# HKU-BAL/MegaPath-Nano

Measured on AMD Instinct MI355X. Metric: Gbp/min ONT reads aligned+species-assigned vs RefSeq, 1/2/4/8 MI355X, higher is better.
Workload: dtype int32

## Files before the change

### megapath_nano_amd/csrc/align.hip

```cpp
#include "map_types.h"
#include "ext_kernels.h"
#include "fin_kernels.h"
#include "stitch_kernels.h"
#include "plan_kernels.h"
#include "hit_kernels.h"
#include "mapper_internal.h"
#include "../../include/mpn_map.h"
#include "../../include/mpn_ssw.h"

#include <algorithm>
#include <condition_variable>
#include <deque>
#include <math.h>
#include <stdio.h>
#include <string.h>
#include <thread>
#include <pthread.h>
#include <time.h>
#include <atomic>
#include <functional>
#include <mutex>
#include <stdlib.h>
#include <string>
#include <vector>
// ... 762 lines not shown
    int nj = nj_cap;
    WallTimer wt;
    Slot &SL = *tl_slot;
    const int strip_scores = ext_strip_scores_ok(opt->a, -opt->b, -opt->sc_ambi, opt->q + opt->e, opt->q2 + opt->e2) ? 1 : 0;
    ExtParams prm;
    prm.sc_mch = (int8_t)opt->a; prm.sc_mis = (int8_t)-opt->b; prm.sc_n = (int8_t)-opt->sc_ambi;
    prm.q = (int8_t)opt->q; prm.e = (int8_t)opt->e; prm.q2 = (int8_t)opt->q2; prm.e2 = (int8_t)opt->e2; prm.zdrop_thres = opt->zdrop;
    prm.zdrop_inv = opt->zdrop_inv; prm.max_gap = opt->max_gap;
    const size_t order_cap = (size_t)nj + (size_t)N_STRIP * 8 + 16;
    if (SL.pool_sizes.ensure((size_t)nj * sizeof(JobSizes) + 16) || SL.pool_buckets.ensure((size_t)2 * N_BUCKETS * 4 + sizeof(LayoutTotals) + 16) ||
        SL.pool_order.ensure(order_cap * 4) || SL.pin_res.ensure(sizeof(LayoutTotals) + 96) ||
        SL.pool_redo_ids.ensure((size_t)nj * 4 + 16) || SL.pool_probes.ensure((size_t)nj * sizeof(InvProbe) + 16))
        return -1;
    struct { ExtJob *p; } d_jobs{dv.jobs};
    JobSizes *d_sizes = SL.pool_sizes.as<JobSizes>();
    int32_t *d_bcnt = SL.pool_buckets.as<int32_t>(), *d_bcur = d_bcnt + N_BUCKETS;
    LayoutTotals *d_tot = reinterpret_cast<LayoutTotals *>(d_bcnt + 2 * N_BUCKETS);
    struct { int32_t *p; } d_order{SL.pool_order.as<int32_t>()};
    {
        ZeroList z{};
        zero_list_push(z, d_bcnt, (size_t)2 * N_BUCKETS * 4 + sizeof(LayoutTotals));
        zero_list_push(z, dv.used + 1, 8);
        zero_list_push(z, dv.used + 5, 8);
        zero_list_push(z, dv.used + 7, 8);
        MPN_HIP_CHECK(zero_regions(z, st));
    }
    const int lay_grid = std::max(1, std::min((nj + 255) / 256, 256));
    EvTimer evl(st);
    static const bool tiled_on = []() { const char *e = getenv("MPN_TILED"); return !e || atoi(e) != 0; }();
    static const int tile_pick = []() { const char *e = getenv("MPN_TILE_CLASS"); return e ? std::min(std::max(atoi(e), 0), N_TILE_CLASS - 1) : -1; }();
    hipLaunchKernelGGL(job_classify_kernel, dim3(lay_grid), dim3(256), 0, st, d_jobs.p, d_nj, strip_scores, prm, g_force_kernel ? g_force_kernel : (tiled_on ? 0 : 7),
                       tile_pick, d_sizes, d_bcnt, d_tot);
    hipLaunchKernelGGL(job_scan_kernel, dim3(1), dim3(1024), 0, st, d_sizes, d_nj, (const int32_t *)d_bcnt, d_bcur, d_tot, d_order.p);
    hipLaunchKernelGGL(job_layout_kernel, dim3(lay_grid), dim3(256), 0, st, d_jobs.p, d_nj, (const JobSizes *)d_sizes, d_bcur, d_order.p);
    MPN_HIP_CHECK(hipGetLastError());
    LayoutTotals *h_tot = SL.pin_res.as<LayoutTotals>();
    evl.mark(56);
    MPN_HIP_CHECK(hipMemcpyAsync(h_tot, d_tot, sizeof(LayoutTotals), hipMemcpyDeviceToHost, st));
    MPN_HIP_CHECK(stream_sync(st));
    evl.resolve();
    const LayoutTotals T = *h_tot;
    nj = T.n_jobs;
    dv.n_jobs = nj;
    if (nj == 0) return 0;
    if (T.too_large) { set_error("DP window too large for LDS staging (%d x %d)", T.tl_q, T.tl_t); return -4; }
    if (!dv.compact) {
// ... 123 lines not shown
    EvTimer ev(st);
    if (!SL.ev_b) {
        MPN_HIP_CHECK(hipEventCreateWithFlags(&SL.ev_b, hipEventDisableTiming));
        MPN_HIP_CHECK(hipEventCreateWithFlags(&SL.ev_c, hipEventDisableTiming));
    }
    auto on_side = [](int l) { return (l >= L_WG && l < L_STRIP) || l >= L_BAND + 8; };
    bool have_tiles = false;
    for (int l = L_TILE; l < N_LISTS; ++l) have_tiles = have_tiles || cnt[l] > 0;
    bool have_side = false;
    for (int l = 0; l < L_TILE; ++l) have_side = have_side || (on_side(l) && cnt[l] > 0);
    hipStream_t extra[2] = {nullptr, nullptr};
    const int n_extra = st.try_extra((int)have_side + (int)have_tiles, extra);
    if (have_side || have_tiles) ++g_stats[n_extra ? STAT_SIDE_LEASED : STAT_SIDE_OWN];
    const hipStream_t main_st = st;
    const hipStream_t side_st = have_side && n_extra > 0 ? extra[0] : main_st;
    const hipStream_t tile_st = have_tiles && n_extra > (int)have_side ? extra[(int)have_side] : main_st;
    for (int l = L_TILE; l < N_LISTS && have_tiles; ++l)
        if (launch_list(l, d_order.p + base[l], cnt[l], tile_st)) return -1;
    for (int l = L_TILE - 1; l >= 0; --l)
        if (on_side(l) && launch_list(l, d_order.p + base[l], cnt[l], side_st)) return -1;
    const int side_lo[2] = {base[L_WG], base[L_BAND + 8]}, side_hi[2] = {base[L_STRIP], base[L_TILE]};
    const int tile_lo[2] = {base[L_TILE], 0}, tile_hi[2] = {base[N_LISTS], 0};
    const int main_lo[2] = {0, base[L_STRIP]}, main_hi[2] = {base[L_WG], base[L_BAND + 8]};
    auto bt_ztest = [&](const int *lo, const int *hi, hipStream_t s, bool timed) -> int {
        for (int k = 0; k < 2; ++k) {
            const int n = hi[k] - lo[k];
            if (n > 0) hipLaunchKernelGGL(ext_bt_kernel, dim3((n + 63) / 64), dim3(64), 0, s, d_jobs.p, d_order.p + lo[k], n, P.p, OFF.p, CIG.p, d_compact, d_used, d_res.p);
        }
        MPN_HIP_CHECK(hipGetLastError());
        if (timed) ev.mark(25);
        for (int k = 0; k < 2; ++k) {
            const int n = hi[k] - lo[k];
            if (n > 0) hipLaunchKernelGGL(ext_ztest_kernel, dim3((n + 63) / 64), dim3(64), 0, s, d_jobs.p, d_order.p + lo[k], n, prm, d_reads, d_read_off, d_read_len, rv, CIG.p, d_res.p,
                                          d_redo_ids, d_used + 1, d_probes, d_used + 5);
        }
        MPN_HIP_CHECK(hipGetLastError());
        if (timed) ev.mark(26);
        return 0;
    };
    if (have_tiles) {
        if (bt_ztest(tile_lo, tile_hi, tile_st, false)) return -1;
        if (tile_st != main_st) MPN_HIP_CHECK(hipEventRecord(SL.ev_c, tile_st));
    }
    if (bt_ztest(side_lo, side_hi, side_st, false)) return -1;
    if (side_st != main_st) MPN_HIP_CHECK(hipEventRecord(SL.ev_b, side_st));
    for (int l = N_LISTS - 1; l >= 0; --l) {
        if (on_side(l)) continue;
        if (l == L_BAND - 1) ev.mark(15);
        if (l >= L_STRIP && l < L_BAND) {
            if (l == L_STRIP + 48) { if (launch_list(l, nullptr, 1, main_st)) return -1; ev.mark(57); }
            else if (l == L_STRIP) { if (launch_list(l, nullptr, 1, main_st)) return -1; ev.mark(9, 38); }
        } else if (launch_list(l, d_order.p + base[l], cnt[l], main_st)) return -1;
    }
    ev.mark(15);
    if (bt_ztest(main_lo, main_hi, main_st, true)) return -1;
    if (side_st != main_st) MPN_HIP_CHECK(hipStreamWaitEvent(main_st, SL.ev_b, 0));
    if (tile_st != main_st) MPN_HIP_CHECK(hipStreamWaitEvent(main_st, SL.ev_c, 0));
    unsigned long long *h_used = reinterpret_cast<unsigned long long *>(reinterpret_cast<char *>(SL.pin_res.p) + ((sizeof(LayoutTotals) + 15) & ~(size_t)15));
    MPN_HIP_CHECK(hipMemcpyAsync(h_used, d_used, 64, hipMemcpyDeviceToHost, st));
    wt.stop_into(g_stats[28]);
    MPN_HIP_CHECK(stream_sync(st));
    wt.stop_into(g_stats[29]);
    if (h_used[7]) {
        g_stats[STAT_TILE_GIVEUPS] += (int64_t)h_used[7];
        set_error("%llu tiled DP windows gave up waiting for their hand-off", (unsigned long long)h_used[7]);
        return -1;
    }
    std::vector<int32_t> redo((size_t)h_used[1]);
    const int n_probe = (int)h_used[5];
    if (!redo.empty() || n_probe) {
        std::vector<ExtJob> jobs((size_t)nj);
        std::vector<InvProbe> probes((size_t)n_probe);
        if (SL.pin_order.ensure(redo.size() * 4 + 16)) return -1;
        if (!redo.empty()) MPN_HIP_CHECK(hipMemcpyAsync(SL.pin_order.p, d_redo_ids, redo.size() * 4, hipMemcpyDeviceToHost, st));
        MPN_HIP_CHECK(hipMemcpyAsync(jobs.data(), d_jobs.p, (size_t)nj * sizeof(ExtJob), hipMemcpyDeviceToHost, st));
        if (n_probe) MPN_HIP_CHECK(hipMemcpyAsync(probes.data(), d_probes, (size_t)n_probe * sizeof(InvProbe), hipMemcpyDeviceToHost, st));
        MPN_HIP_CHECK(stream_sync(st));
        if (!redo.empty()) memcpy(redo.data(), SL.pin_order.p, redo.size() * 4);
        std::vector<uint8_t> is_inv((size_t)nj, 0);
        if (n_probe) {
            std::sort(probes.begin(), probes.end(), [](const InvProbe &x, const InvProbe &y) { return x.jid < y.jid; });
            std::vector<LocalHit> hits((size_t)n_probe, LocalHit{0, -1, -1});
            if (hs) {
                std::vector<std::vector<int8_t>> qv((size_t)n_probe), tv;
                std::vector<RefIv> iv((size_t)n_probe);
// ... 35 lines not shown
                const int64_t n_r = (int64_t)jb.qlen + jb.tlen - 1;
                pack_off[k] = -1 - p2_tot;
                p2_tot += ((bv >= 0 ? n_r * (128 << bv) : n_r * jb.n_col) + 15) & ~(int64_t)15;
            } else pack_off[k] = jb.p_off;
        }
        if (nr > 0) {
            if (SL.pool_P2.ensure((size_t)p2_tot + 16)) return -1;
            const int64_t p2_base = (int64_t)(SL.pool_P2.as<uint8_t>() - P.p);
            for (int k = 0; k < nr; ++k) if (pack_off[k] < 0) pack_off[k] = p2_base + (-1 - pack_off[k]);
            if (SL.pool_redo.ensure(pack.size() * 4)) return -1;
            struct { int32_t *p; } d_redo{SL.pool_redo.as<int32_t>()};
            MPN_HIP_CHECK(hipMemcpyAsync(d_redo.p, pack.data(), pack.size() * 4, hipMemcpyHostToDevice, st));
            hipLaunchKernelGGL(ext_redo_patch_kernel, dim3((nr + 255) / 256), dim3(256), 0, st, d_jobs.p, d_redo.p, d_redo.p + nr, d_redo.p + 2 * nr,
                               reinterpret_cast<const int64_t *>(d_redo.p + off_p), d_redo.p + 3 * nr, opt->zdrop_inv, nr);
            MPN_HIP_CHECK(hipGetLastError());
            ev.skip();
            for (int lo = 0; lo < nr;) {
                int hi = lo;
                while (hi < nr && redo_list_of(redo[hi]) == redo_list_of(redo[lo])) ++hi;
                if (launch_list(redo_list_of(redo[lo]), d_redo.p + lo, hi - lo, st)) return -1;
                lo = hi;
            }
            ev.mark(15);
            hipLaunchKernelGGL(ext_bt_kernel, dim3((nr + 63) / 64), dim3(64), 0, st, d_jobs.p, d_redo.p, nr, P.p, OFF.p, CIG.p, d_compact, d_used, d_res.p);
            MPN_HIP_CHECK(hipGetLastError());
            ev.mark(25);
            MPN_HIP_CHECK(stream_sync(st));
        }
    }
    ev.resolve();
    wt.stop_into(g_stats[30]);
    return 0;
}

static int run_jobs(const RefView &rv, const mpn_map_opt *opt, int nj_cap, const uint8_t *d_reads, const int64_t *d_read_off,
                    const int32_t *d_read_len, DevRound &out, const HostSeqs *hs, StreamLease &st, bool block_zeroed = false) {
    static const int64_t budget = []() { const char *e = getenv("MPN_DP_BUDGET"); return e ? std::max<int64_t>(1 << 20, atoll(e)) : (int64_t)40 << 30; }();
    Slot &SL = *tl_slot;
    if (SL.pool_res.ensure((size_t)nj_cap * sizeof(ExtRes) + 16) || SL.pool_used.ensure(128)) return -1;
    out.jobs = SL.pool_jobs.as<ExtJob>(); out.res = SL.pool_res.as<ExtRes>(); out.compact = nullptr;
    out.used = SL.pool_used.as<unsigned long long>();
    if (!block_zeroed) {
        MPN_HIP_CHECK(hipMemsetAsync(out.used, 0, 24, st));
        MPN_HIP_CHECK(hipMemsetAsync(out.used + 5, 0, 24, st));
    }
    const int rc = run_job_group(rv, opt, nj_cap, out.used + 3, out, d_reads, d_read_off, d_read_len, budget, hs, st);
    if (rc != 1) return rc;
// ... 1133 lines not shown
    std::vector<int64_t> ns, ne;
    pack_2bit(tcodes, ttot, words, ns, ne);
    DevBuf<int32_t> d_qlen;
    if (d_reads.upload(ascii.data(), ascii.size(), st) || d_ref.upload(words.data(), words.size(), st) || d_ns.upload(ns.data(), ns.size(), st) ||
        d_ne.upload(ne.data(), ne.size(), st) || d_qoff.upload(q_off, n, st) ||
        d_qlen.upload(q_len, n, st) || d_toff.upload(t_off, n, st))
        return -1;
    std::vector<ExtJob> jobs(n);
    for (int i = 0; i < n; ++i) {
        ExtJob &j = jobs[i];
        memset(&j, 0, sizeof(j));
        j.read = i; j.rid = i; j.rev = 0; j.qs = 0; j.qlen = q_len[i]; j.ts = 0; j.tlen = t_len[i]; j.reversed = 0;
        j.w = w[i]; j.zdrop = zdrop[i]; j.end_bonus = end_bonus[i]; j.flag = flag[i];
    }
    g_force_kernel = force_kernel;
    mpn_map_opt o2 = *opt;
    o2.zdrop = 0x3fffffff;
    DevRound dv;
    for (ExtJob &j : jobs) { j.strip_s = 1; j.cls = -1; }
    if (tl_slot->pool_jobs.ensure((size_t)n * sizeof(ExtJob) + 16)) return -1;
    MPN_HIP_CHECK(hipMemcpy(tl_slot->pool_jobs.p, jobs.data(), (size_t)n * sizeof(ExtJob), hipMemcpyHostToDevice));
    {
        const unsigned long long cnt = (unsigned long long)n;
        if (tl_slot->pool_used.ensure(64)) return -1;
        MPN_HIP_CHECK(hipMemcpy(tl_slot->pool_used.as<unsigned long long>() + 3, &cnt, 8, hipMemcpyHostToDevice));
    }
    StreamLease sl(st);
    const int rc = run_jobs(RefView{d_ref.p, d_toff.p, d_ns.p, d_ne.p, (int32_t)ns.size()}, &o2, n, d_reads.p, d_qoff.p, d_qlen.p, dv, nullptr, sl);
    g_force_kernel = 0;
    if (rc) return rc;
    std::vector<ExtRes> res((size_t)n);
    unsigned long long h_used = 0;
    MPN_HIP_CHECK(hipMemcpy(res.data(), dv.res, (size_t)n * sizeof(ExtRes), hipMemcpyDeviceToHost));
    MPN_HIP_CHECK(hipMemcpy(&h_used, dv.used, 8, hipMemcpyDeviceToHost));
    std::vector<uint32_t> cig((size_t)h_used + 1);
    if (h_used) MPN_HIP_CHECK(hipMemcpy(cig.data(), dv.compact, (size_t)h_used * 4, hipMemcpyDeviceToHost));
    int64_t used = 0;
    for (int i = 0; i < n; ++i) {
        const ExtRes &e = res[i];
        int32_t *o = out9 + (size_t)i * 9;
        o[0] = e.max; o[1] = e.zdropped; o[2] = e.max_q; o[3] = e.max_t; o[4] = e.mqe; o[5] = e.mqe_t; o[6] = e.score; o[7] = e.reach_end;
        o[8] = e.n_cigar;
        cig_off[i] = used;
        if (used + e.n_cigar > cigar_cap) return -3;
        if (e.n_cigar) memcpy(cigar_pool + used, cig.data() + e.cig_pos, (size_t)e.n_cigar * 4);
        used += e.n_cigar;
    }
// ... 3 lines not shown
```

### megapath_nano_amd/csrc/ext_kernels.h

```cpp
#pragma once
#include "mpn_common.h"
#include "map_types.h"

namespace mpn {

enum { EZ_APPROX_MAX = 0x02, EZ_RIGHT = 0x08, EZ_EXTZ_ONLY = 0x40, EZ_REV_CIGAR = 0x80 };

struct ExtJob {
    int32_t read;
    int32_t rid;
    int32_t rev;
    int32_t qs, qlen;
    int32_t ts, tlen;
    int32_t reversed;
    int32_t w, zdrop, end_bonus, flag;
    int64_t p_off;
    int64_t row_off;
    int64_t cig_off;
    int32_t n_col;
    int32_t state_mode;
    int64_t state_off;
    int32_t layout;
    int32_t qstride;
    int32_t strip_s;
// ... 1265 lines not shown
            res[jid] = out;
        }
    }
}

template <int S, int NW>
__global__ __launch_bounds__(64 * NW) void ext_dp_tile_kernel(const ExtJob *__restrict__ jobs, const int32_t *__restrict__ order, int n_jobs,
                                                              ExtParams prm, const uint8_t *__restrict__ reads,
                                                              const int64_t *__restrict__ read_off, const int32_t *__restrict__ read_len,
                                                              RefView rv, uint8_t *__restrict__ P, int8_t *__restrict__ gstate, ExtRes *__restrict__ res,
                                                              unsigned long long *__restrict__ n_failed) {
    extern __shared__ __attribute__((aligned(16))) uint8_t smem[];
    const int jid = order[blockIdx.x];
    const ExtJob jb = jobs[jid];
#define MPN_TB(EX, RT) ext_tile_body<S, NW, EX, RT>(jb, jid, prm, reads, read_off, read_len, rv, P, gstate, res, smem, n_failed)
    if (jb.flag & EZ_APPROX_MAX) MPN_TB(false, false);
    else if (jb.flag & EZ_RIGHT) MPN_TB(true, true);
    else MPN_TB(true, false);
#undef MPN_TB
}



__global__ __launch_bounds__(64) void ext_bt_kernel(const ExtJob *__restrict__ jobs, const int32_t *__restrict__ order, int n_jobs,
                                                    const uint8_t *__restrict__ P, const int32_t *__restrict__ OFF,
                                                    uint32_t *__restrict__ CIG, uint32_t *__restrict__ COMPACT,
                                                    unsigned long long *__restrict__ compact_used, ExtRes *__restrict__ res) {
    const int k = blockIdx.x * blockDim.x + threadIdx.x;
    const int jid = k < n_jobs ? order[k] : -1;
    const bool live = jid >= 0;
    ExtJob jb = jobs[live ? jid : 0];
    ExtRes r = res[live ? jid : 0];
    const bool walk = live && r.do_bt;
    if (live && !r.do_bt) res[jid].cig_pos = 0;
    if (!walk) { jb.qlen = jb.tlen = 1; r.bt_i = r.bt_j = -1; }
    const int n_col = jb.n_col, n_r = jb.qlen + jb.tlen - 1;
    const uint8_t *p = P + jb.p_off;
    const int32_t *off = OFF + 2 * jb.row_off, *off_end = off + n_r;
    const bool rowmajor = jb.layout == 1;
    const bool rank_is_op = (jb.flag & EZ_RIGHT) != 0;
    const bool byslot = jb.layout == 2;
    const bool tiled = jb.layout == 3;
    TileGeom tg{};
    int tg_tile = -1;
    const int bw = jb.w < 0 ? (jb.tlen > jb.qlen ? jb.tlen : jb.qlen) : jb.w;
    const bool rev_cigar = (jb.flag & EZ_REV_CIGAR) != 0;
// ... 2 lines not shown
    uint32_t *cbeg = cend - cap;
    int n = 0, i = r.bt_i, j = r.bt_j, state = 0;
    uint32_t cur_op = 0xf, cur_len = 0;
#define MPN_FLUSH() do { if (cur_len) { if (rev_cigar) cbeg[n] = cur_len << 4 | cur_op; else cend[-1 - n] = cur_len << 4 | cur_op; ++n; } } while (0)
#define MPN_PUSHOP(OP, LEN) do { if ((uint32_t)(OP) == cur_op) cur_len += (LEN); else { MPN_FLUSH(); cur_op = (OP); cur_len = (LEN); } } while (0)
    constexpr int BT_AHEAD = 8;
    while (i >= 0 && j >= 0) {
        const int rr = i + j;
        int force_state = -1, tmp;
        if (rowmajor) {
            if (state == 0) {
                uint8_t ahead[BT_AHEAD];
#pragma unroll
                for (int k = 0; k < BT_AHEAD; ++k) {
                    const int ii = i - k, jj = j - k;
                    ahead[k] = (ii >= 0 && jj >= 0) ? p[(int64_t)(jj + ii / jb.strip_s) * jb.qstride + ii] : (uint8_t)0xff;
                }
                int k = 0;
                tmp = 0;
#pragma unroll
                for (int q = 0; q < BT_AHEAD; ++q) {
                    if (k != q) continue;
                    if (i - q < 0 || j - q < 0) continue;
                    int b = ahead[q];
                    if (!rank_is_op) b = (b & ~7) | (4 - (b & 7));
                    if ((b & 7) == 0) ++k; else tmp = b;
                }
                if (k > 0) { MPN_PUSHOP(0, (uint32_t)k); i -= k; j -= k; }
                if (k == BT_AHEAD || i < 0 || j < 0) continue;
            } else {
                tmp = p[(int64_t)(j + i / jb.strip_s) * jb.qstride + i];
                if (!rank_is_op) tmp = (tmp & ~7) | (4 - (tmp & 7));
            }
        }
        else if (tiled) {
            int st = 0, en = jb.tlen - 1;
            if (st < rr - jb.qlen + 1) st = rr - jb.qlen + 1;
            if (en > rr) en = rr;
            if (st < (rr - bw + 1) >> 1) st = (rr - bw + 1) >> 1;
            if (en > (rr + bw) >> 1) en = (rr + bw) >> 1;
            if (i < st) force_state = 2;
            if (i > en) force_state = 1;
            tmp = 0;
            if (force_state < 0) {
                const int tile = i / (64 * jb.strip_s);
                if (tile != tg_tile) { tg = tile_geom(tile, jb.qlen, jb.tlen, bw, jb.strip_s); tg_tile = tile; }
                const int lt = i - tg.T0;
                tmp = p[tg.base + (int64_t)((j - tg.jlo) + lt / jb.strip_s) * tg.W + lt];
                if (!rank_is_op) tmp = (tmp & ~7) | (4 - (tmp & 7));
            }
        }
        else if (byslot) {
            int st = 0, en = jb.tlen - 1;
            if (st < rr - jb.qlen + 1) st = rr - jb.qlen + 1;
            if (en > rr) en = rr;
            if (st < (rr - bw + 1) >> 1) st = (rr - bw + 1) >> 1;
            if (en > (rr + bw) >> 1) en = (rr + bw) >> 1;
            if (i < st) force_state = 2;
            if (i > en) force_state = 1;
            tmp = force_state < 0 ? p[(int64_t)rr * jb.qstride + (i & (jb.qstride - 1))] : 0;
        } else {
            if (i < off[rr]) force_state = 2;
            if (i > off_end[rr]) force_state = 1;
            tmp = force_state < 0 ? p[(int64_t)rr * n_col + i - off[rr]] : 0;
        }
        if (state == 0) state = tmp & 7;
        else if (!(tmp >> (state + 2) & 1)) state = 0;
        if (state == 0) state = tmp & 7;
        if (force_state >= 0) state = force_state;
        if (state == 0) { MPN_PUSHOP(0, 1); --i; --j; }
        else if (state == 1 || state == 3) { MPN_PUSHOP(2, 1); --i; }
        else { MPN_PUSHOP(1, 1); --j; }
    }
    if (walk) {
        if (i >= 0) MPN_PUSHOP(2, (uint32_t)(i + 1));
        if (j >= 0) MPN_PUSHOP(1, (uint32_t)(j + 1));
        MPN_FLUSH();
    }
#undef MPN_PUSHOP
#undef MPN_FLUSH
    const int lane = threadIdx.x & 63;
    int incl = n;
#pragma unroll
    for (int d = 1; d < 64; d <<= 1) { const int o = __shfl_up(incl, d); if (lane >= d) incl += o; }
    const int total = __shfl(incl, 63);
    unsigned long long base = 0;
    if (lane == 0 && total) base = atomicAdd(compact_used, (unsigned long long)total);
    base = (unsigned long long)__shfl((long long)base, 0);
    if (walk) {
        const unsigned long long pos = base + (unsigned long long)(incl - n);
        const uint32_t *src = rev_cigar ? cbeg : cend - n;
        for (int q = 0; q < n; ++q) COMPACT[pos + q] = src[q];
        res[jid].n_cigar = n;
        res[jid].cig_pos = (int64_t)pos;
    }
}

__global__ __launch_bounds__(64) void ext_ztest_kernel(const ExtJob *__restrict__ jobs, const int32_t *__restrict__ order, int n_jobs,
                                                       ExtParams prm, const uint8_t *__restrict__ reads,
                                                       const int64_t *__restrict__ read_off, const int32_t *__restrict__ read_len,
                                                       RefView rv,
                                                       const uint32_t *__restrict__ CIG, ExtRes *__restrict__ res,
                                                       int32_t *__restrict__ redo_ids, unsigned long long *__restrict__ n_redo,
                                                       InvProbe *__restrict__ probes, unsigned long long *__restrict__ n_probe) {
    const int k = blockIdx.x * blockDim.x + threadIdx.x;
    if (k >= n_jobs) return;
    const int jid = order[k];
    if (jid < 0) return;
    const ExtJob jb = jobs[jid];
    if (!(jb.flag & EZ_APPROX_MAX)) return;
    auto report = [&](int z) {
        res[jid].zcode = z;
        if (z) redo_ids[atomicAdd(n_redo, 1ULL)] = jid;
    };
    const ExtRes r = res[jid];
    const int zmin = prm.zdrop_thres < prm.zdrop_inv ? prm.zdrop_thres : prm.zdrop_inv;
    const uint32_t *cig = CIG + jb.cig_off - r.n_cigar;
    if ((jb.layout == 1 || jb.layout == 3) && r.do_bt && !r.zdropped) {
// ... 29 lines not shown
                } else { mx = score; max_i = i + l; max_j = j + l; }
            }
            i += len; j += len;
        } else if (op == 1 || op == 2) {
            score -= prm.q + prm.e * (int)len;
            if (op == 1) j += len; else i += len;
            if (score < mx) {
                const int li = i - max_i, lj = j - max_j, diff = li > lj ? li - lj : lj - li;
                const int z = mx - score - diff * prm.e;
                if (z > max_zdrop) { max_zdrop = z; p00 = max_i; p01 = max_j; p10 = i; p11 = j; }
            } else { mx = score; max_i = i; max_j = j; }
        }
    }
    const int over = max_zdrop > prm.zdrop_thres ? 1 : 0;
    const int q_len = p11 - p01, t_len = p10 - p00;
    if (max_zdrop > prm.zdrop_inv && q_len < prm.max_gap && t_len < prm.max_gap && q_len > 0 && t_len > 0) {
        res[jid].zcode = over;
        probes[atomicAdd(n_probe, 1ULL)] = InvProbe{jid, p00, p01, p10, p11, over};
        return;
    }
    report(over);
}

}
```

### megapath_nano_amd/csrc/mapper_internal.h

```cpp
#pragma once
#include "mpn_common.h"
#include "map_types.h"
#include "queue_lease.h"

#include <atomic>
#include <chrono>
#include <time.h>
#include <mutex>
#include <stdint.h>
#include <stdlib.h>
#include <string.h>
#include <string>
#include <vector>

struct mpn_map_opt_s;


struct mpn_index {
    int k = 15, w = 10;
    int32_t n_seq = 0;
    std::vector<std::string> names;
    std::vector<int32_t> lens;
    std::vector<int64_t> seq_off;
    std::vector<uint32_t> h_seq2;
// ... 28 lines not shown
    DevBuf<unsigned long long> used;
};

struct ReadSketch {
    DevBuf<int64_t> mz_off;
    DevBuf<u128> mz;
    int64_t n_mz = 0;
    int k = 0, w = 0;
    bool valid = false;
};

struct HostChains {
    std::vector<int64_t> n_anchor, chain_off, b_off;
    std::vector<int64_t> n_chained, u_pos, b_pos;
    std::vector<int32_t> n_chain, rep_len;
    const uint64_t *u_all = nullptr;
    const u128 *b_all = nullptr;
    const ChainRec *rec_all = nullptr;
    int64_t n_pool_chains = 0;
    void read_chains(int i, uint64_t *u_out, u128 *b_out) const;
    void chain_order(int i, int32_t *order, int64_t *src) const;
};

constexpr int MPN_NSTATS = 73;
constexpr int STAT_LEASE_WAIT = 65;
constexpr int STAT_SIDE_LEASED = 66, STAT_SIDE_OWN = 67;
constexpr int STAT_TILE_CLASS = 68, STAT_TILE_GIVEUPS = 72;
extern thread_local int64_t g_stats[MPN_NSTATS];

void pack_2bit(const uint8_t *codes, int64_t n, std::vector<uint32_t> &words, std::vector<int64_t> &ns, std::vector<int64_t> &ne);

hipError_t stream_sync(hipStream_t st);

struct QueueStreams {
    LeasePool pool;
    std::vector<hipStream_t> st;
    explicit QueueStreams(int q) : pool(q), st((size_t)q, nullptr) {}
};
QueueStreams *queue_streams(int dev);

class StreamLease {
  public:
    explicit StreamLease(QueueStreams *qs) : qs_(qs) {}
    explicit StreamLease(hipStream_t fixed) : fixed_(fixed) {}
    StreamLease(const StreamLease &) = delete;
    StreamLease &operator=(const StreamLease &) = delete;
    ~StreamLease() { release(); }
    hipStream_t get() {
        if (!qs_) return fixed_;
        if (n_ == 0) n_ = qs_->pool.acquire(1, id_, &g_stats[STAT_LEASE_WAIT]);
// ... 121 lines not shown
```

### megapath_nano_amd/mapper.py

```python
import ctypes as ct
import os

import numpy as np

from . import _ffi


class MapOpt(ct.Structure):
    _fields_ = [('k', ct.c_int32), ('w', ct.c_int32), ('mid_occ_frac', ct.c_float), ('mid_occ', ct.c_int32),
                ('max_gap', ct.c_int32), ('bw', ct.c_int32), ('max_chain_skip', ct.c_int32), ('max_chain_iter', ct.c_int32),
                ('min_cnt', ct.c_int32), ('min_chain_score', ct.c_int32), ('mask_level', ct.c_float),
                ('pri_ratio', ct.c_float), ('best_n', ct.c_int32), ('max_join_long', ct.c_int32),
                ('max_join_short', ct.c_int32), ('min_join_flank_sc', ct.c_int32), ('min_join_flank_ratio', ct.c_float),
                ('a', ct.c_int32), ('b', ct.c_int32), ('q', ct.c_int32), ('e', ct.c_int32), ('q2', ct.c_int32),
                ('e2', ct.c_int32), ('sc_ambi', ct.c_int32), ('zdrop', ct.c_int32), ('zdrop_inv', ct.c_int32),
                ('end_bonus', ct.c_int32), ('min_dp_max', ct.c_int32), ('min_ksw_len', ct.c_int32),
                ('max_clip_ratio', ct.c_float), ('max_sw_mat', ct.c_int64), ('with_cigar', ct.c_int32),
                ('seed', ct.c_uint32), ('host_threads', ct.c_int32), ('out_sam', ct.c_int32)]


COL_NAMES = ('read_idx', 'qs', 'qe', 'rev', 'rid', 'rs', 're', 'mlen', 'blen', 'mapq', 'nm', 'as_', 'primary')


class AlnCols(ct.Structure):
# ... 537 lines not shown
    _ffi.check(rc, 'mpn_ext_dp_batch')
    keys = ('max', 'zdropped', 'max_q', 'max_t', 'mqe', 'mqe_t', 'score', 'reach_end', 'n_cigar')
    res = []
    for i in range(n):
        d = {k: int(out[i, j]) for j, k in enumerate(keys)}
        d['cigar'] = [int(x) for x in pool[coff[i]:coff[i] + d['n_cigar']]]
        res.append(d)
    return res


STAT_NAMES = {0: 'bases', 1: 'minimizers', 2: 'anchors', 3: 'chains', 4: 'dp_jobs', 5: 'dp_cells', 6: 'alignments',
              7: 'dp_rounds', 8: 'second_pass_jobs', 10: 'ev_sketch_ns', 11: 'ev_seed_ns', 12: 'ev_sort_ns',
              13: 'ev_chain_dp_ns', 14: 'ev_chain_bt_ns', 15: 'ev_ext_dp_ns', 25: 'ev_ext_bt_ns', 26: 'ev_ext_ztest_ns',
              16: 'wall_h2d_ns', 17: 'wall_seed_chain_ns', 18: 'wall_d2h_chains_ns', 19: 'wall_host_hits_ns',
              20: 'wall_host_plan_ns', 21: 'wall_ext_stage_ns', 22: 'wall_host_stitch_ns', 23: 'wall_host_final_ns',
              24: 'wall_total_ns', 27: 'wall_ext_host_prep_ns', 28: 'wall_ext_enqueue_ns', 29: 'wall_ext_gpu_wait_ns',
              30: 'wall_ext_finish_ns', 9: 'ev_ext_strip_ns', 31: 'strip_cells', 32: 'sub_batches',
              33: 'k_sketch_count_ns', 34: 'k_sketch_fill_ns', 35: 'k_seed_lookup_ns', 36: 'k_seed_fill_ns',
              37: 'k_chain_dp_ns', 38: 'k_strip16_ns', 39: 'k_strip32_ns', 40: 'k_strip64_ns', 41: 'strip16_cells',
              42: 'strip32_cells', 43: 'strip64_cells', 44: 'sort_records_moved', 45: 'anchors_kept', 46: 'k_compact_ns', 47: 'k_sort_msd_ns', 48: 'k_sort_chunk_ns', 49: 'k_sort_radix_ns',
              50: 'k_seed_filter_ns', 51: 'anchors_emitted', 52: 'k_finish_ns', 53: 'cigar_ops', 54: 'k_stitch_ns', 55: 'k_plan_ns', 56: 'k_layout_ns', 57: 'k_xstrip_ns', 58: 'xstrip_cells', 59: 'anchors_squeezed', 60: 'workers_shed', 61: 'workers', 62: 'k_hit_select_ns', 63: 'reads_hits_on_host',
              64: 'tile_windows', 65: 'wall_lease_wait_ns', 66: 'ext_groups_side_leased', 67: 'ext_groups_side_own',
              68: 'tile_windows_1w_s16', 69: 'tile_windows_s4_nw8', 70: 'tile_windows_s8_nw4', 71: 'tile_windows_s4_nw16',
              72: 'tile_wait_giveups'}


def last_stats():
    n = max(STAT_NAMES) + 1
    s = np.zeros(n, dtype=np.int64)
    _bind().mpn_map_last_stats_ex(s.ctypes.data, n)
    return {name: int(s[i]) for i, name in STAT_NAMES.items()}
```

Measured before the change: 13.74.

## Add wave-parallel traceback and z-drop test kernels for long extension windows

Adds wavefront-per-job variants of the extension traceback and z-drop test kernels. The traceback stages a 64x64 patch of the direction matrix into shared memory and uses ballots to advance runs of identical moves. The z-drop test processes CIGAR ops across lanes and uses prefix scans over match runs. By default the side and tiled job groups use the wave kernels and the main group keeps the one-thread-per-job kernels, with an env var to force either mode. This targets the serial per-thread walk over long alignments, at the cost of more blocks, shared-memory staging and a few new counters.

```diff
diff --git a/megapath_nano_amd/csrc/align.hip b/megapath_nano_amd/csrc/align.hip
--- a/megapath_nano_amd/csrc/align.hip
+++ b/megapath_nano_amd/csrc/align.hip
@@ -808,6 +808,7 @@
         zero_list_push(z, d_bcnt, (size_t)2 * N_BUCKETS * 4 + sizeof(LayoutTotals));
         zero_list_push(z, dv.used + 1, 8);
         zero_list_push(z, dv.used + 5, 8);
+        zero_list_push(z, dv.used + 8, 16);
         zero_list_push(z, dv.used + 7, 8);
         MPN_HIP_CHECK(zero_regions(z, st));
     }
@@ -977,28 +978,39 @@
     const int side_lo[2] = {base[L_WG], base[L_BAND + 8]}, side_hi[2] = {base[L_STRIP], base[L_TILE]};
     const int tile_lo[2] = {base[L_TILE], 0}, tile_hi[2] = {base[N_LISTS], 0};
     const int main_lo[2] = {0, base[L_STRIP]}, main_hi[2] = {base[L_WG], base[L_BAND + 8]};
-    auto bt_ztest = [&](const int *lo, const int *hi, hipStream_t s, bool timed) -> int {
-        for (int k = 0; k < 2; ++k) {
-            const int n = hi[k] - lo[k];
-            if (n > 0) hipLaunchKernelGGL(ext_bt_kernel, dim3((n + 63) / 64), dim3(64), 0, s, d_jobs.p, d_order.p + lo[k], n, P.p, OFF.p, CIG.p, d_compact, d_used, d_res.p);
-        }
+    static const int walk_mode = []() {
+        const char *e = getenv("MPN_EXT_WALK");
+        return !e || !strcmp(e, "auto") ? 0 : !strcmp(e, "lane") ? 1 : !strcmp(e, "wave") ? 2 : 0;
+    }();
+    auto launch_bt = [&](const int32_t *ord, int n, hipStream_t s, bool wave) {
+        if (n <= 0) return;
+        if (wave) hipLaunchKernelGGL(ext_bt_wave_kernel, dim3(n), dim3(64), 0, s, d_jobs.p, ord, n, P.p, OFF.p, CIG.p, d_compact, d_used, d_res.p, d_used + 8);
+        else hipLaunchKernelGGL(ext_bt_kernel, dim3((n + 63) / 64), dim3(64), 0, s, d_jobs.p, ord, n, P.p, OFF.p, CIG.p, d_compact, d_used, d_res.p);
+    };
+    auto bt_ztest = [&](const int *lo, const int *hi, hipStream_t s, bool timed, bool wave) -> int {
+        for (int k = 0; k < 2; ++k) launch_bt(d_order.p + lo[k], hi[k] - lo[k], s, wave);
         MPN_HIP_CHECK(hipGetLastError());
         if (timed) ev.mark(25);
         for (int k = 0; k < 2; ++k) {
             const int n = hi[k] - lo[k];
-            if (n > 0) hipLaunchKernelGGL(ext_ztest_kernel, dim3((n + 63) / 64), dim3(64), 0, s, d_jobs.p, d_order.p + lo[k], n, prm, d_reads, d_read_off, d_read_len, rv, CIG.p, d_res.p,
-                                          d_redo_ids, d_used + 1, d_probes, d_used + 5);
+            if (n <= 0) continue;
+            if (wave) hipLaunchKernelGGL(ext_ztest_wave_kernel, dim3(n), dim3(64), 0, s, d_jobs.p, d_order.p + lo[k], n, prm, d_reads, d_read_off, d_read_len, rv, CIG.p, d_res.p,
+                                         d_redo_ids, d_used + 1, d_probes, d_used + 5, d_used + 9);
+            else hipLaunchKernelGGL(ext_ztest_kernel, dim3((n + 63) / 64), dim3(64), 0, s, d_jobs.p, d_order.p + lo[k], n, prm, d_reads, d_read_off, d_read_len, rv, CIG.p, d_res.p,
+                                    d_redo_ids, d_used + 1, d_probes, d_used + 5);
         }
         MPN_HIP_CHECK(hipGetLastError());
         if (timed) ev.mark(26);
         return 0;
     };
+    if (have_side || have_tiles) ev.mark(15);
     if (have_tiles) {
-        if (bt_ztest(tile_lo, tile_hi, tile_st, false)) return -1;
+        if (bt_ztest(tile_lo, tile_hi, tile_st, false, walk_mode != 1)) return -1;
         if (tile_st != main_st) MPN_HIP_CHECK(hipEventRecord(SL.ev_c, tile_st));
     }
-    if (bt_ztest(side_lo, side_hi, side_st, false)) return -1;
+    if (bt_ztest(side_lo, side_hi, side_st, false, walk_mode != 1)) return -1;
     if (side_st != main_st) MPN_HIP_CHECK(hipEventRecord(SL.ev_b, side_st));
+    if (have_side || have_tiles) ev.mark(STAT_EV_WALK_LONG);
     for (int l = N_LISTS - 1; l >= 0; --l) {
         if (on_side(l)) continue;
         if (l == L_BAND - 1) ev.mark(15);
@@ -1008,14 +1020,16 @@
         } else if (launch_list(l, d_order.p + base[l], cnt[l], main_st)) return -1;
     }
     ev.mark(15);
-    if (bt_ztest(main_lo, main_hi, main_st, true)) return -1;
+    if (bt_ztest(main_lo, main_hi, main_st, true, walk_mode == 2)) return -1;
     if (side_st != main_st) MPN_HIP_CHECK(hipStreamWaitEvent(main_st, SL.ev_b, 0));
     if (tile_st != main_st) MPN_HIP_CHECK(hipStreamWaitEvent(main_st, SL.ev_c, 0));
     unsigned long long *h_used = reinterpret_cast<unsigned long long *>(reinterpret_cast<char *>(SL.pin_res.p) + ((sizeof(LayoutTotals) + 15) & ~(size_t)15));
-    MPN_HIP_CHECK(hipMemcpyAsync(h_used, d_used, 64, hipMemcpyDeviceToHost, st));
+    MPN_HIP_CHECK(hipMemcpyAsync(h_used, d_used, 80, hipMemcpyDeviceToHost, st));
     wt.stop_into(g_stats[28]);
     MPN_HIP_CHECK(stream_sync(st));
     wt.stop_into(g_stats[29]);
+    g_stats[STAT_WALK_WAVE] += (int64_t)h_used[8];
+    g_stats[STAT_WALK_WAVE_FAILED] += (int64_t)h_used[9];
     if (h_used[7]) {
         g_stats[STAT_TILE_GIVEUPS] += (int64_t)h_used[7];
         set_error("%llu tiled DP windows gave up waiting for their hand-off", (unsigned long long)h_used[7]);
@@ -1097,7 +1111,8 @@
                 lo = hi;
             }
             ev.mark(15);
-            hipLaunchKernelGGL(ext_bt_kernel, dim3((nr + 63) / 64), dim3(64), 0, st, d_jobs.p, d_redo.p, nr, P.p, OFF.p, CIG.p, d_compact, d_used, d_res.p);
+            launch_bt(d_redo.p, nr, st, walk_mode == 2);
+            if (walk_mode == 2) g_stats[STAT_WALK_WAVE] += nr;
             MPN_HIP_CHECK(hipGetLastError());
             ev.mark(25);
             MPN_HIP_CHECK(stream_sync(st));
@@ -2277,7 +2292,7 @@
     MPN_HIP_CHECK(hipMemcpy(tl_slot->pool_jobs.p, jobs.data(), (size_t)n * sizeof(ExtJob), hipMemcpyHostToDevice));
     {
         const unsigned long long cnt = (unsigned long long)n;
-        if (tl_slot->pool_used.ensure(64)) return -1;
+        if (tl_slot->pool_used.ensure(128)) return -1;
         MPN_HIP_CHECK(hipMemcpy(tl_slot->pool_used.as<unsigned long long>() + 3, &cnt, 8, hipMemcpyHostToDevice));
     }
     StreamLease sl(st);
diff --git a/megapath_nano_amd/csrc/ext_kernels.h b/megapath_nano_amd/csrc/ext_kernels.h
--- a/megapath_nano_amd/csrc/ext_kernels.h
+++ b/megapath_nano_amd/csrc/ext_kernels.h
@@ -1311,6 +1311,28 @@
 
 
 
+__device__ __forceinline__ void ext_bt_band(int rr, int qlen, int tlen, int bw, int &st, int &en) {
+    st = 0; en = tlen - 1;
+    if (st < rr - qlen + 1) st = rr - qlen + 1;
+    if (en > rr) en = rr;
+    if (st < (rr - bw + 1) >> 1) st = (rr - bw + 1) >> 1;
+    if (en > (rr + bw) >> 1) en = (rr + bw) >> 1;
+}
+__device__ __forceinline__ int ext_bt_force(int i, int st, int en) {
+    int force_state = -1;
+    if (i < st) force_state = 2;
+    if (i > en) force_state = 1;
+    return force_state;
+}
+__device__ __forceinline__ int ext_bt_decode(int b, bool rank_is_op) { return rank_is_op ? b : (b & ~7) | (4 - (b & 7)); }
+__device__ __forceinline__ int ext_bt_next_state(int state, int tmp, int force_state) {
+    if (state == 0) state = tmp & 7;
+    else if (!(tmp >> (state + 2) & 1)) state = 0;
+    if (state == 0) state = tmp & 7;
+    if (force_state >= 0) state = force_state;
+    return state;
+}
+
 __global__ __launch_bounds__(64) void ext_bt_kernel(const ExtJob *__restrict__ jobs, const int32_t *__restrict__ order, int n_jobs,
                                                     const uint8_t *__restrict__ P, const int32_t *__restrict__ OFF,
                                                     uint32_t *__restrict__ CIG, uint32_t *__restrict__ COMPACT,
@@ -1359,52 +1381,37 @@
                 for (int q = 0; q < BT_AHEAD; ++q) {
                     if (k != q) continue;
                     if (i - q < 0 || j - q < 0) continue;
-                    int b = ahead[q];
-                    if (!rank_is_op) b = (b & ~7) | (4 - (b & 7));
+                    const int b = ext_bt_decode(ahead[q], rank_is_op);
                     if ((b & 7) == 0) ++k; else tmp = b;
                 }
                 if (k > 0) { MPN_PUSHOP(0, (uint32_t)k); i -= k; j -= k; }
                 if (k == BT_AHEAD || i < 0 || j < 0) continue;
             } else {
-                tmp = p[(int64_t)(j + i / jb.strip_s) * jb.qstride + i];
-                if (!rank_is_op) tmp = (tmp & ~7) | (4 - (tmp & 7));
+                tmp = ext_bt_decode(p[(int64_t)(j + i / jb.strip_s) * jb.qstride + i], rank_is_op);
             }
         }
         else if (tiled) {
-            int st = 0, en = jb.tlen - 1;
-            if (st < rr - jb.qlen + 1) st = rr - jb.qlen + 1;
-            if (en > rr) en = rr;
-            if (st < (rr - bw + 1) >> 1) st = (rr - bw + 1) >> 1;
-            if (en > (rr + bw) >> 1) en = (rr + bw) >> 1;
-            if (i < st) force_state = 2;
-            if (i > en) force_state = 1;
+            int st, en;
+            ext_bt_band(rr, jb.qlen, jb.tlen, bw, st, en);
+            force_state = ext_bt_force(i, st, en);
             tmp = 0;
             if (force_state < 0) {
                 const int tile = i / (64 * jb.strip_s);
                 if (tile != tg_tile) { tg = tile_geom(tile, jb.qlen, jb.tlen, bw, jb.strip_s); tg_tile = tile; }
                 const int lt = i - tg.T0;
-                tmp = p[tg.base + (int64_t)((j - tg.jlo) + lt / jb.strip_s) * tg.W + lt];
-                if (!rank_is_op) tmp = (tmp & ~7) | (4 - (tmp & 7));
+                tmp = ext_bt_decode(p[tg.base + (int64_t)((j - tg.jlo) + lt / jb.strip_s) * tg.W + lt], rank_is_op);
             }
         }
         else if (byslot) {
-            int st = 0, en = jb.tlen - 1;
-            if (st < rr - jb.qlen + 1) st = rr - jb.qlen + 1;
-            if (en > rr) en = rr;
-            if (st < (rr - bw + 1) >> 1) st = (rr - bw + 1) >> 1;
-            if (en > (rr + bw) >> 1) en = (rr + bw) >> 1;
-            if (i < st) force_state = 2;
-            if (i > en) force_state = 1;
+            int st, en;
+            ext_bt_band(rr, jb.qlen, jb.tlen, bw, st, en);
+            force_state = ext_bt_force(i, st, en);
             tmp = force_state < 0 ? p[(int64_t)rr * jb.qstride + (i & (jb.qstride - 1))] : 0;
         } else {
-            if (i < off[rr]) force_state = 2;
-            if (i > off_end[rr]) force_state = 1;
+            force_state = ext_bt_force(i, off[rr], off_end[rr]);
             tmp = force_state < 0 ? p[(int64_t)rr * n_col + i - off[rr]] : 0;
         }
-        if (state == 0) state = tmp & 7;
-        else if (!(tmp >> (state + 2) & 1)) state = 0;
-        if (state == 0) state = tmp & 7;
-        if (force_state >= 0) state = force_state;
+        state = ext_bt_next_state(state, tmp, force_state);
         if (state == 0) { MPN_PUSHOP(0, 1); --i; --j; }
         else if (state == 1 || state == 3) { MPN_PUSHOP(2, 1); --i; }
         else { MPN_PUSHOP(1, 1); --j; }
@@ -1431,6 +1438,141 @@
         res[jid].n_cigar = n;
         res[jid].cig_pos = (int64_t)pos;
     }
+}
+
+__global__ __launch_bounds__(64) void ext_bt_wave_kernel(const ExtJob *__restrict__ jobs, const int32_t *__restrict__ order, int n_jobs,
+                                                         const uint8_t *__restrict__ P, const int32_t *__restrict__ OFF,
+                                                         uint32_t *__restrict__ CIG, uint32_t *__restrict__ COMPACT,
+                                                         unsigned long long *__restrict__ compact_used, ExtRes *__restrict__ res,
+                                                         unsigned long long *__restrict__ n_windows) {
+    constexpr int PR = 64, PC = 64;
+    __shared__ uint8_t patch[PR * PC];
+    __shared__ int32_t s_lim[2][PR];
+    const int lane = threadIdx.x;
+    if ((int)blockIdx.x >= n_jobs) return;
+    const int jid = order[blockIdx.x];
+    if (jid < 0) return;
+    if (lane == 0) atomicAdd(n_windows, 1ULL);
+    const ExtJob jb = jobs[jid];
+    const ExtRes r = res[jid];
+    if (!r.do_bt) { if (lane == 0) res[jid].cig_pos = 0; return; }
+    const int layout = jb.layout, S = jb.strip_s > 0 ? jb.strip_s : 1, R = 64 * S;
+    const int n_col = jb.n_col, n_r = jb.qlen + jb.tlen - 1;
+    const uint8_t *p = P + jb.p_off;
+    const int32_t *off = OFF + 2 * jb.row_off, *off_end = off + n_r;
+    const bool rank_is_op = (jb.flag & EZ_RIGHT) != 0 || layout == 0 || layout == 2;
+    const int bw = jb.w < 0 ? (jb.tlen > jb.qlen ? jb.tlen : jb.qlen) : jb.w;
+    const bool rev_cigar = (jb.flag & EZ_REV_CIGAR) != 0;
+    uint32_t *cend = CIG + jb.cig_off;
+    const int cap = jb.qlen + jb.tlen + 2;
+    uint32_t *cbeg = cend - cap;
+    int n = 0, i = r.bt_i, j = r.bt_j, state = 0;
+    uint32_t cur_op = 0xf, cur_len = 0;
+#define MPN_FLUSH() do { if (cur_len) { if (lane == 0) { if (rev_cigar) cbeg[n] = cur_len << 4 | cur_op; else cend[-1 - n] = cur_len << 4 | cur_op; } ++n; } } while (0)
+#define MPN_PUSHOP(OP, LEN) do { if ((uint32_t)(OP) == cur_op) cur_len += (LEN); else { MPN_FLUSH(); cur_op = (OP); cur_len = (LEN); } } while (0)
+    TileGeom tg{};
+    int tg_tile = -1;
+    bool p_valid = false;
+    int p_mtop = 0, p_itop = 0;
+    auto major_of = [&](int ii, int jj) -> int {
+        if (layout == 1) return jj + ii / S;
+        if (layout == 3) return (jj - tg.jlo) + (ii - tg.T0) / S;
+        return ii + jj;
+    };
+    auto patch_slot = [&](int ii, int jj) -> int {
+        if (!p_valid || ii < 0 || jj < 0) return -1;
+        if (layout == 3 && ii < tg.T0) return -1;
+        const int mrel = p_mtop - major_of(ii, jj), irel = p_itop - ii;
+        return (mrel >= 0 && mrel < PR && irel >= 0 && irel < PC) ? mrel * PC + irel : -1;
+    };
+    auto force_of = [&](int ii, int jj) -> int {
+        if (layout == 1) return -1;
+        if (layout == 0) { const int mrel = p_mtop - (ii + jj); return ext_bt_force(ii, s_lim[0][mrel], s_lim[1][mrel]); }
+        int st, en;
+        ext_bt_band(ii + jj, jb.qlen, jb.tlen, bw, st, en);
+        return ext_bt_force(ii, st, en);
+    };
+    auto stage = [&]() {
+        __syncthreads();
+        p_valid = true; p_itop = i; p_mtop = major_of(i, j);
+        const int ii = p_itop - lane;
+        if (layout == 0) {
+            const int m = p_mtop - lane;
+            s_lim[0][lane] = m >= 0 ? off[m] : 0;
+            s_lim[1][lane] = m >= 0 ? off_end[m] : -1;
+            __syncthreads();
+        }
+        uint8_t v[PR];
+#pragma unroll
+        for (int q = 0; q < PR; ++q) {
+            const int m = p_mtop - q;
+            bool ok = m >= 0 && ii >= 0;
+            int64_t a = 0;
+            if (layout == 1) a = (int64_t)m * jb.qstride + ii;
+            else if (layout == 3) { ok = ok && ii >= tg.T0; a = tg.base + (int64_t)m * tg.W + (ii - tg.T0); }
+            else if (layout == 2) a = (int64_t)m * jb.qstride + (ii & (jb.qstride - 1));
+            else {
+                const int lo = s_lim[0][q], hi = s_lim[1][q];
+                ok = ok && ii >= lo && ii <= hi && ii - lo < n_col;
+                a = (int64_t)m * n_col + (ii - lo);
+            }
+            v[q] = ok ? p[a] : (uint8_t)0;
+        }
+#pragma unroll
+        for (int q = 0; q < PR; ++q) patch[q * PC + lane] = v[q];
+        __syncthreads();
+    };
+    while (i >= 0 && j >= 0) {
+        if (layout == 0 && !(p_valid && p_mtop - (i + j) >= 0 && p_mtop - (i + j) < PR)) stage();
+        const int force_state = force_of(i, j);
+        if (force_state >= 0) {
+            const int di = force_state == 1 ? 1 : 0, dj = 1 - di;
+            const int ii = i - lane * di, jj = j - lane * dj;
+            bool go = ii >= 0 && jj >= 0;
+            if (go && layout == 0) go = p_mtop - (ii + jj) < PR;
+            go = go && force_of(ii, jj) == force_state;
+            const unsigned long long mask = __ballot(go);
+            const int k = ~mask ? __builtin_ctzll(~mask) : 64;
+            state = force_state;
+            MPN_PUSHOP(di ? 2 : 1, (uint32_t)k);
+            i -= k * di; j -= k * dj;
+            continue;
+        }
+        if (layout == 3 && i / R != tg_tile) { tg_tile = i / R; tg = tile_geom(tg_tile, jb.qlen, jb.tlen, bw, S); p_valid = false; }
+        if (patch_slot(i, j) < 0) stage();
+        {
+            const int di = (state == 2 || state == 4) ? 0 : 1, dj = (state == 1 || state == 3) ? 0 : 1;
+            const int ii = i - lane * di, jj = j - lane * dj;
+            int slot = patch_slot(ii, jj);
+            if (slot >= 0 && force_of(ii, jj) >= 0) slot = -1;
+            const int b = ext_bt_decode(patch[slot >= 0 ? slot : 0], rank_is_op);
+            const bool go = slot >= 0 && (state == 0 ? (b & 7) == 0 : (b >> (state + 2) & 1) != 0);
+            const unsigned long long mask = __ballot(go);
+            const int k = ~mask ? __builtin_ctzll(~mask) : 64;
+            if (k > 0) {
+                MPN_PUSHOP(state == 0 ? 0 : di ? 2 : 1, (uint32_t)k);
+                i -= k * di; j -= k * dj;
+                continue;
+            }
+        }
+        state = ext_bt_next_state(state, ext_bt_decode(patch[patch_slot(i, j)], rank_is_op), -1);
+        if (state == 0) { MPN_PUSHOP(0, 1); --i; --j; }
+        else if (state == 1 || state == 3) { MPN_PUSHOP(2, 1); --i; }
+        else { MPN_PUSHOP(1, 1); --j; }
+    }
+    if (i >= 0) MPN_PUSHOP(2, (uint32_t)(i + 1));
+    if (j >= 0) MPN_PUSHOP(1, (uint32_t)(j + 1));
+    MPN_FLUSH();
+#undef MPN_PUSHOP
+#undef MPN_FLUSH
+    unsigned long long base = 0;
+    if (lane == 0 && n) base = atomicAdd(compact_used, (unsigned long long)n);
+    base = (unsigned long long)__shfl((long long)base, 0);
+    __threadfence_block();
+    __syncthreads();
+    const uint32_t *src = rev_cigar ? cbeg : cend - n;
+    for (int q = lane; q < n; q += 64) COMPACT[base + q] = src[q];
+    if (lane == 0) { res[jid].n_cigar = n; res[jid].cig_pos = (int64_t)base; }
 }
 
 __global__ __launch_bounds__(64) void ext_ztest_kernel(const ExtJob *__restrict__ jobs, const int32_t *__restrict__ order, int n_jobs,
@@ -1506,4 +1648,147 @@
     report(over);
 }
 
-}
+__global__ __launch_bounds__(64) void ext_ztest_wave_kernel(const ExtJob *__restrict__ jobs, const int32_t *__restrict__ order, int n_jobs,
+                                                            ExtParams prm, const uint8_t *__restrict__ reads,
+                                                            const int64_t *__restrict__ read_off, const int32_t *__restrict__ read_len,
+                                                            RefView rv,
+                                                            const uint32_t *__restrict__ CIG, ExtRes *__restrict__ res,
+                                                            int32_t *__restrict__ redo_ids, unsigned long long *__restrict__ n_redo,
+                                                            InvProbe *__restrict__ probes, unsigned long long *__restrict__ n_probe,
+                                                            unsigned long long *__restrict__ n_failed) {
+    constexpr int ZW = 1024;
+    __shared__ uint8_t s_t[ZW], s_q[ZW];
+    const int lane = threadIdx.x;
+    if ((int)blockIdx.x >= n_jobs) return;
+    const int jid = order[blockIdx.x];
+    if (jid < 0) return;
+    const ExtJob jb = jobs[jid];
+    if (!(jb.flag & EZ_APPROX_MAX)) return;
+    const ExtRes r = res[jid];
+    const int zmin = prm.zdrop_thres < prm.zdrop_inv ? prm.zdrop_thres : prm.zdrop_inv;
+    const int n_cig = r.n_cigar;
+    const uint32_t *cig = CIG + jb.cig_off - n_cig;
+    if ((jb.layout == 1 || jb.layout == 3) && r.do_bt && !r.zdropped) {
+        long long m_cols = 0, extra = 0;
+        for (int c = lane; c < n_cig; c += 64) {
+            const uint32_t op = cig[c] & 0xf;
+            const int64_t len = cig[c] >> 4;
+            if (op == 0) m_cols += len;
+            else if (op == 1 || op == 2) {
+                const int64_t w1 = prm.q + prm.e * len, w2 = prm.q2 + prm.e2 * len;
+                extra += w1 - (w1 < w2 ? w1 : w2);
+            }
+        }
+#pragma unroll
+        for (int d = 32; d >= 1; d >>= 1) { m_cols += __shfl_xor(m_cols, d); extra += __shfl_xor(extra, d); }
+        if ((int64_t)prm.sc_mch * m_cols - r.score + extra <= zmin) { if (lane == 0) res[jid].zcode = 0; return; }
+    }
+    const int64_t roff = read_off[jb.read];
+    const int32_t rlen = read_len[jb.read];
+    const int64_t g0 = rv.seq_off[jb.rid] + jb.ts;
+    int32_t score = 0, mx = INT32_MIN, max_i = -1, max_j = -1, i = 0, j = 0, max_zdrop = 0;
+    int32_t p00 = -1, p01 = -1, p10 = -1, p11 = -1;
+    int t_base = 0, q_base = 0;
+    bool staged = false;
+    auto stage = [&](int ti, int qi) {
+        __syncthreads();
+        staged = true;
+        t_base = (int)(((g0 + ti) & ~(int64_t)15) - g0);
+        q_base = qi;
+        {
+            const int64_t gw = g0 + t_base + 16 * lane;
+            uint32_t word = 0;
+            bool slow = false;
+            if (gw < g0 + jb.tlen) {
+                word = rv.seq2[gw >> 4];
+                if (rv.n_runs > 0) {
+                    int lo = 0, hi = rv.n_runs;
+                    while (lo < hi) { const int mid = (lo + hi) >> 1; if (rv.nrun_s[mid] <= gw + 15) lo = mid + 1; else hi = mid; }
+                    slow = lo > 0 && rv.nrun_e[lo - 1] > gw;
+                }
+            }
+#pragma unroll
+            for (int b = 0; b < 16; ++b) {
+                const int64_t g = gw + b;
+                int c = (int)((word >> (2 * b)) & 3u);
+                if (g < g0 || g >= g0 + jb.tlen) c = 4;
+                else if (slow) c = ref_code(rv, g);
+                s_t[16 * lane + b] = (uint8_t)c;
+            }
+        }
+#pragma unroll
+        for (int u = 0; u < ZW / 64; ++u) {
+            const int x = q_base + 64 * u + lane;
+            s_q[64 * u + lane] = x < jb.qlen ? ext_qbase(reads, roff, rlen, jb.rev, jb.qs + x) : (uint8_t)4;
+        }
+        __syncthreads();
+    };
+    for (int c0 = 0; c0 < n_cig; c0 += 64) {
+        const uint32_t mine = c0 + lane < n_cig ? cig[c0 + lane] : 0u;
+        const int nc = n_cig - c0 < 64 ? n_cig - c0 : 64;
+        for (int c = 0; c < nc; ++c) {
+            const uint32_t word = (uint32_t)__shfl((int)mine, c);
+            const uint32_t op = word & 0xf, len = word >> 4;
+            if (op == 0) {
+                for (uint32_t l0 = 0; l0 < len; l0 += 64) {
+                    const int cnt = len - l0 < 64 ? (int)(len - l0) : 64, ci = i + (int)l0, cj = j + (int)l0;
+                    if (!staged || ci < t_base || ci + cnt > t_base + ZW || cj < q_base || cj + cnt > q_base + ZW) stage(ci, cj);
+                    const int ct = s_t[(ci - t_base + lane) & (ZW - 1)], cq = s_q[(cj - q_base + lane) & (ZW - 1)];
+                    const int sc1 = lane < cnt ? ((ct == 4 || cq == 4) ? prm.sc_n : ct == cq ? prm.sc_mch : prm.sc_mis) : 0;
+                    int sc = sc1;
+#pragma unroll
+                    for (int d = 1; d < 64; d <<= 1) { const int o = __shfl_up(sc, d); if (lane >= d) sc += o; }
+                    sc += score;
+                    int mv = lane < cnt ? sc : INT32_MIN, mi = lane;
+#pragma unroll
+                    for (int d = 1; d < 64; d <<= 1) {
+                        const int ov = __shfl_up(mv, d), oi = __shfl_up(mi, d);
+                        if (lane >= d && ov > mv) { mv = ov; mi = oi; }
+                    }
+                    int bv = __shfl_up(mv, 1), bi = __shfl_up(mi, 1);
+                    if (lane == 0) { bv = INT32_MIN; bi = -1; }
+                    const bool in_run = bi >= 0 && bv >= mx;
+                    const int d0 = (ci - max_i) - (cj - max_j), diff = in_run ? 0 : d0 < 0 ? -d0 : d0;
+                    const int before = in_run ? bv : mx;
+                    int z = 0;
+                    if (lane < cnt && sc < before) z = before - sc - diff * prm.e;
+                    int zbest = z;
+#pragma unroll
+                    for (int d = 32; d >= 1; d >>= 1) { const int o = __shfl_xor(zbest, d); zbest = o > zbest ? o : zbest; }
+                    if (zbest > max_zdrop) {
+                        const int src = __builtin_ctzll(__ballot(z == zbest));
+                        const int s_in = __shfl((int)in_run, src), s_bi = __shfl(bi, src);
+                        max_zdrop = zbest;
+                        p00 = s_in ? ci + s_bi : max_i; p01 = s_in ? cj + s_bi : max_j;
+                        p10 = ci + src; p11 = cj + src;
+                    }
+                    const int ev = __shfl(mv, cnt - 1), ei = __shfl(mi, cnt - 1);
+                    score = __shfl(sc, cnt - 1);
+                    if (ev >= mx) { mx = ev; max_i = ci + ei; max_j = cj + ei; }
+                }
+                i += len; j += len;
+            } else if (op == 1 || op == 2) {
+                score -= prm.q + prm.e * (int)len;
+                if (op == 1) j += len; else i += len;
+                if (score < mx) {
+                    const int li = i - max_i, lj = j - max_j, diff = li > lj ? li - lj : lj - li;
+                    const int z = mx - score - diff * prm.e;
+                    if (z > max_zdrop) { max_zdrop = z; p00 = max_i; p01 = max_j; p10 = i; p11 = j; }
+                } else { mx = score; max_i = i; max_j = j; }
+            }
+        }
+    }
+    if (lane != 0) return;
+    const int over = max_zdrop > prm.zdrop_thres ? 1 : 0;
+    const int q_len = p11 - p01, t_len = p10 - p00;
+    if (max_zdrop > prm.zdrop_inv && q_len < prm.max_gap && t_len < prm.max_gap && q_len > 0 && t_len > 0) {
+        res[jid].zcode = over;
+        probes[atomicAdd(n_probe, 1ULL)] = InvProbe{jid, p00, p01, p10, p11, over};
+        atomicAdd(n_failed, 1ULL);
+        return;
+    }
+    res[jid].zcode = over;
+    if (over) { redo_ids[atomicAdd(n_redo, 1ULL)] = jid; atomicAdd(n_failed, 1ULL); }
+}
+
+}
diff --git a/megapath_nano_amd/csrc/mapper_internal.h b/megapath_nano_amd/csrc/mapper_internal.h
--- a/megapath_nano_amd/csrc/mapper_internal.h
+++ b/megapath_nano_amd/csrc/mapper_internal.h
@@ -74,10 +74,11 @@
     void chain_order(int i, int32_t *order, int64_t *src) const;
 };
 
-constexpr int MPN_NSTATS = 73;
+constexpr int MPN_NSTATS = 76;
 constexpr int STAT_LEASE_WAIT = 65;
 constexpr int STAT_SIDE_LEASED = 66, STAT_SIDE_OWN = 67;
 constexpr int STAT_TILE_CLASS = 68, STAT_TILE_GIVEUPS = 72;
+constexpr int STAT_WALK_WAVE = 73, STAT_EV_WALK_LONG = 74, STAT_WALK_WAVE_FAILED = 75;
 extern thread_local int64_t g_stats[MPN_NSTATS];
 
 void pack_2bit(const uint8_t *codes, int64_t n, std::vector<uint32_t> &words, std::vector<int64_t> &ns, std::vector<int64_t> &ne);
diff --git a/megapath_nano_amd/mapper.py b/megapath_nano_amd/mapper.py
--- a/megapath_nano_amd/mapper.py
+++ b/megapath_nano_amd/mapper.py
@@ -583,7 +583,9 @@
               50: 'k_seed_filter_ns', 51: 'anchors_emitted', 52: 'k_finish_ns', 53: 'cigar_ops', 54: 'k_stitch_ns', 55: 'k_plan_ns', 56: 'k_layout_ns', 57: 'k_xstrip_ns', 58: 'xstrip_cells', 59: 'anchors_squeezed', 60: 'workers_shed', 61: 'workers', 62: 'k_hit_select_ns', 63: 'reads_hits_on_host',
               64: 'tile_windows', 65: 'wall_lease_wait_ns', 66: 'ext_groups_side_leased', 67: 'ext_groups_side_own',
               68: 'tile_windows_1w_s16', 69: 'tile_windows_s4_nw8', 70: 'tile_windows_s8_nw4', 71: 'tile_windows_s4_nw16',
-              72: 'tile_wait_giveups'}
+              72: 'tile_wait_giveups',
+              73: 'walk_wave_windows', 74: 'ev_ext_walk_long_ns',
+              75: 'walk_wave_failed'}
 
 
 def last_stats():
```

After: 14.87 (median of 6 runs). +8.2%, better.
